# isl-org/adaptive-surface-reconstruction

Hardware: AMD Instinct MI355X
Metric: input points/sec to signed implicit values (higher is better)
Workload: dtype f32 via bf16x3 (24-bit operands, f32 accumulate)

## Files before the change

adaptive-surface-reconstruction_amd/csrc/asr_common.h:

```cpp
#pragma once
#include <hip/hip_runtime.h>

#include <cstdint>
#include <cstdio>
#include <map>
#include <string>
#include <tuple>
#include <vector>

#include "../../include/asr_hip.h"

typedef uint64_t u64;
typedef int64_t i64;
typedef uint32_t u32;

struct Arena {
    struct Slab {
        char* base;
        size_t size, used;
    };
    std::vector<Slab> slabs;
    size_t min_slab = size_t(256) << 20;
    size_t cap = 0;

    void* alloc(size_t bytes) {
        bytes = (bytes + 255) & ~size_t(255);
        if (bytes == 0) bytes = 256;
        for (auto& s : slabs)
            if (s.size - s.used >= bytes) {
                void* p = s.base + s.used;
                s.used += bytes;
                return p;
            }
        size_t sz = bytes > min_slab ? bytes : min_slab;
        if (cap && reserved() + sz > cap) return nullptr;
        void* p = nullptr;
        if (hipMalloc(&p, sz) != hipSuccess) return nullptr;
        slabs.push_back({(char*)p, sz, bytes});
        return p;
    }
    void reset() {
        for (auto& s : slabs) s.used = 0;
    }
    size_t reserved() const {
        size_t t = 0;
        for (auto& s : slabs) t += s.size;
        return t;
    }
    void release() {
        for (auto& s : slabs) (void)hipFree(s.base);
        slabs.clear();
    }
};

struct ArenaMark {
    std::vector<size_t> used;
};
static inline void arena_mark(const Arena& a, ArenaMark& m) {
    m.used.clear();
    for (auto& s : a.slabs) m.used.push_back(s.used);
}
static inline void arena_rewind(Arena& a, const ArenaMark& m) {
    for (size_t i = 0; i < a.slabs.size(); ++i) a.slabs[i].used = i < m.used.size() ? m.used[i] : 0;
}

struct GridDev {
    i64 v = 0, p = 0;
    u64* keys = nullptr;
    float* centers = nullptr;
    float* sizes = nullptr;
    int32_t* nidx = nullptr;
    uint8_t* nkidx = nullptr;
    i64* nrs = nullptr;
    int32_t* up_idx = nullptr;
    uint8_t* up_kidx = nullptr;
    i64* up_rs = nullptr;
    int32_t* down_idx = nullptr;
    uint8_t* down_kidx = nullptr;
    i64* down_rs = nullptr;
    int32_t* perm_nb = nullptr;
    int32_t* perm_up = nullptr;
    int32_t* perm_down = nullptr;
};

struct AsrOptions {
    i64 sconv_min_blocks = 2816;
    i64 sconv16_min_blocks = 1024;
    i64 sconv_wide_min = 2048;
    i64 row_segment = 524288;
    i64 search_hash_level = -1;
    i64 knn_deep = 1;
    i64 knn_cells = 1;
    i64 plan_arena = 0;
    i64 sconv_plan = 1;
    i64 row_ranked = 1;
    i64 row_lpt = 1;
    i64 overlap = 1;
    i64 cconv_valu = 0;
    i64 build_search = 1;
    i64 shard_geometry = -1;
    i64 shard_timing = 0;
    i64 search_priority = 2;
    i64 search_half = 1;
    i64 early_cells = 1;
    i64 early_sort = 1;
    i64 arena_cap_mb = 0;
    i64 inject_failure = 0;
    i64 sconv_split_min_rows = 2048;
    i64 sconv_split_rows = 32768;
};

struct asr_conv_plan_view {
    const uint4* hdr;
    const int32_t* pool;
    i64 groups;
    unsigned pool_bytes;
};
struct asr_conv_plan {
    uint4* hdr = nullptr;
    int32_t* pool = nullptr;
    i64 groups = 0, groups_pad = 0, blocks = 0;
    i64* offs = nullptr;
    const int32_t* nidx = nullptr;
    const uint8_t* kidx = nullptr;
    const i64* rs = nullptr;
    const int32_t* perm = nullptr;
    i64 num_out = 0;
    int K = 0;
    bool usable() const { return hdr && blocks * 64 < (i64(1) << 32) - 65536; }
    asr_conv_plan_view view() const { return {hdr, pool, groups, (unsigned)(blocks * 64)}; }
};

struct AsrPointIndex {
    bool valid = false;
    const float* pts = nullptr;
    const float* radii = nullptr;
    i64 n = 0;
    int lsort = 0;
    float4* sorted = nullptr;
    int32_t* ids = nullptr;
    int32_t* rank = nullptr;
    float* srad = nullptr;
    u64* codes = nullptr;
    u64* tab_keys = nullptr;
    u64 tab_mask = 0;
    int32_t* tab_start = nullptr;
    int32_t* tab_end = nullptr;
    int tab_lmin = 0, tab_lmax = -1, tab_lhash = 0, tab_grow = 0;
};

struct asr_hip_context {
    hipStream_t stream = nullptr;
    std::string err;
    AsrOptions opt;
    std::map<const void*, asr_conv_plan> conv_plans;
    std::map<std::string, i64> sconv_launches;
    ArenaMark build_mark;
    bool build_mark_ok = false;
    Arena persist;
    Arena scratch;
    Arena plan_arena;
    uint64_t plan_arena_epoch = 0;
    u64* nodes = nullptr;
    u64* leaves = nullptr;
    i64 num_nodes = 0, num_leaves = 0;
    asr_octree_frame frame;
    asr_implicit_sizes sizes;
    GridDev grids[ASR_NUM_GRIDS];
    int32_t* agg_idx = nullptr;
    float* agg_dist = nullptr;
    float* agg_compat = nullptr;
    i64* agg_rs = nullptr;
    int32_t* agg_spos = nullptr;
    const float4* agg_sorted = nullptr;
    bool has_search = false;
    bool build_sharded = false;
    const int32_t* agg_rows = nullptr;
    i64 agg_nq = 0;
    const float* agg_qcenters = nullptr;
    const float* agg_qsizes = nullptr;
    AsrPointIndex pindex;
    i64 shard_prefix_hint = 0;
    int search_extras = 0;
    int leaf_lmin = -1, leaf_lmax = -1;
    float* values = nullptr;
    float* feats1 = nullptr;
    int feats1_width = 0;
    float* importance = nullptr;
    float* code = nullptr;
    bool code_ok = false;
    int code_width = 0;
    int code_scale_sdf = 0;
    float stage_ms[6] = {0, 0, 0, 0, 0, 0};
    hipEvent_t ev[8] = {};
    bool ev_ok = false;
    int* d_flags = nullptr;
    int* d_flags_base = nullptr;
    int flags_next = 0;
    float* d_zeros = nullptr;
    float* split_part = nullptr;
    size_t split_part_bytes = 0;
    unsigned* d_status = nullptr;
    unsigned* d_absmax = nullptr;
    void* radius_state = nullptr;
    void* mesh_state = nullptr;
    std::map<std::string, std::pair<const void*, size_t>> named;
    int device = 0;
    asr_hip_context* aux = nullptr;
    bool aux_stream_owned = false;
    hipEvent_t aux_ev = nullptr;
    hipEvent_t aux_t0 = nullptr, aux_t1 = nullptr;
    bool search_overlapped = false;
    typedef std::tuple<const void*, const void*, i64, i64, i64, i64, int> PackedKey;
    std::map<PackedKey, void*> packed_weights;
    Arena shard_mem;
    unsigned* shard_stage_send = nullptr;
    unsigned* shard_stage_recv = nullptr;
    size_t shard_stage_cap = 0;
    struct asr_shard_state* shard = nullptr;
    bool dry_launch = false;
};

#define ASR_FAIL(ctx, code, ...)                         \
    do {                                                 \
        char _b[512];                                    \
        snprintf(_b, sizeof(_b), __VA_ARGS__);           \
        (ctx)->err = _b;                                 \
        return (code);                                   \
    } while (0)

#define ASR_HIP_CHECK(ctx, expr)                                                            \
    do {                                                                                    \
        hipError_t _e = (expr);                                                             \
        if (_e != hipSuccess)                                                               \
            ASR_FAIL(ctx, ASR_HIP_EHIP, "%s failed: %s (%s:%d)", #expr, hipGetErrorString(_e), \
                     __FILE__, __LINE__);                                                   \
    } while (0)

#define ASR_CHECK_LAUNCH(ctx) ASR_HIP_CHECK(ctx, hipGetLastError())

#define ASR_TRY(expr)               \
    do {                            \
        int _r = (expr);            \
        if (_r != ASR_HIP_OK) return _r; \
    } while (0)

static inline int asr_ctx_zeros(asr_hip_context* ctx, const float** out) {
    if (!ctx->d_zeros) {
        ASR_HIP_CHECK(ctx, hipMalloc((void**)&ctx->d_zeros, 4096));
        ASR_HIP_CHECK(ctx, hipMemsetAsync(ctx->d_zeros, 0, 4096, ctx->stream));
    }
    *out = ctx->d_zeros;
    return ASR_HIP_OK;
}

template <class T>
static inline T* arena_alloc(Arena& a, size_t count) {
    return (T*)a.alloc(count * sizeof(T));
}

static inline unsigned grid_for(i64 n, int block) {
    i64 g = (n + block - 1) / block;
    if (g < 1) g = 1;
    return (unsigned)g;
}

__host__ __device__ static inline u64 asr_dilate21(u64 x) {
    x = (x | (x << 32)) & 0x001F00000000FFFFull;
    x = (x | (x << 16)) & 0x00FF0000FF0000FFull;
    x = (x | (x << 8)) & 0xF00F00F00F00F00Full;
    x = (x | (x << 4)) & 0x30C30C30C30C30C3ull;
    x = (x | (x << 2)) & 0x9249249249249249ull;
    return x;
}
__host__ __device__ static inline u64 asr_compact21(u64 x) {
    x &= 0x1249249249249249ull;
    x = ((x >> 2) | x) & 0x30C30C30C30C30C3ull;
    x = ((x >> 4) | x) & 0xF00F00F00F00F00Full;
    x = ((x >> 8) | x) & 0x00FF0000FF0000FFull;
    x = ((x >> 16) | x) & 0x001F00000000FFFFull;
    x = ((x >> 32) | x) & 0x00000000001FFFFFull;
    return x;
}
// ... 190 lines not shown
```

adaptive-surface-reconstruction_amd/csrc/asr_conv16.hip:

```cpp
#include <type_traits>

#include "asr_common.h"

namespace {

typedef float f32x4 __attribute__((ext_vector_type(4)));
typedef unsigned u32x4 __attribute__((ext_vector_type(4)));
typedef _Float16 f16x8 __attribute__((ext_vector_type(8)));
typedef __bf16 bf16x8 __attribute__((ext_vector_type(8)));
typedef float f32x2 __attribute__((ext_vector_type(2)));
typedef __bf16 bf16x2 __attribute__((ext_vector_type(2)));
typedef uint16_t u16;

constexpr int NBR_LD = 57;

constexpr bool is_bf16x3(int mode) { return mode == ASR_CONV16_BF16X3 || mode == ASR_CONV16_BF16X3_2ACC; }

__device__ inline u16 f32_to_bf16_bits(float x) {
    const f32x2 v = {x, 0.f};
    return (u16)(__builtin_bit_cast(unsigned, __builtin_convertvector(v, bf16x2)) & 0xffffu);
}

__device__ inline u16 f32_to_f16_bits(float x) {
    _Float16 h = (_Float16)x;
// ... 422 lines not shown
            if (SV_EXACT || w_lds[s] >= 0) s_B[buf][w_lds[s]] = st[s];
    };
    constexpr int ESZ = MODE == ASR_CONV16_F16 ? 2 : 4;
    const i64 a_span = a.num_inp > 0 ? ((a.num_inp - 1) * a.inp_ld + cin) * ESZ : 0;
    const bool a_big = a_span > (i64)(OOB_OFF - 4096);
    const __amdgpu_buffer_rsrc_t rs_a =
            __builtin_amdgcn_make_buffer_rsrc((void*)a.inp_features, 0, a_big ? 0 : (int)(unsigned)a_span, RSRC_FLAGS);
    const bool cin_tail = cin % KC != 0;
    int cache_k = -2;
    unsigned cache_off = OOB_OFF;
    const char* cache_row = (const char*)zeros;
    bool cache_valid = false;
    auto gather_a = [&](const int qk, const int qp, u32x4 (&aq)[NJ * AW]) __attribute__((always_inline)) {
        if (qk != cache_k) {
            cache_k = qk;
            const int idx = qk < 0 ? -1 : s_nbr[lrow * NBR_LD + qk];
            cache_valid = idx >= 0;
            cache_off = cache_valid ? (unsigned)idx * (unsigned)(a.inp_ld * ESZ) + (unsigned)(8 * g * ESZ) : OOB_OFF;
            if (a_big) cache_row = (const char*)a.inp_features + (i64)(cache_valid ? idx : 0) * a.inp_ld * ESZ;
        }
        if (!a_big && !cin_tail) {
            const int soff = qp * KC * ESZ;
#pragma unroll
            for (int j = 0; j < NJ; ++j)
#pragma unroll
                for (int h = 0; h < AW; ++h)
                    aq[j * AW + h] = __builtin_amdgcn_raw_buffer_load_b128(rs_a, (int)cache_off + (32 * j + 4 * h) * ESZ,
                                                                           soff, 0);
            return;
        }
#pragma unroll
        for (int j = 0; j < NJ; ++j) {
            const int c = qp * KC + 32 * j + 8 * g;
#pragma unroll
            for (int h = 0; h < AW; ++h) {
                const int cc = c + 4 * h;
                if (a_big) {
                    const void* src = (cache_valid && cc < cin) ? (const void*)(cache_row + (i64)cc * ESZ) : (const void*)zeros;
                    aq[j * AW + h] = *reinterpret_cast<const u32x4*>(src);
                } else {
                    const unsigned vo = cc < cin ? cache_off + (unsigned)((32 * j + 4 * h) * ESZ) : OOB_OFF;
                    aq[j * AW + h] = __builtin_amdgcn_raw_buffer_load_b128(rs_a, (int)vo, qp * KC * ESZ, 0);
                }
            }
        }
    };

    unsigned long long todo1 = bmask;
    int k_cur = bmask ? __builtin_ctzll(bmask) : -1, p_cur = 0;
    int k1 = k_cur, p1 = 0;
    ASR_SEQ_ADVANCE(todo1, k1, p1)
    if (k_cur >= 0) {
        load_panel(k_cur, p_cur, stage0);
        gather_a(k_cur, p_cur, a_q0);
        store_panel(0, stage0);
        load_panel(k1, p1, stage1);
        gather_a(k1, p1, a_q1);
    }
    __syncthreads();
    int buf = 0;
    const int ncol = lane & 15;
    auto step = [&](u32x4 (&aq)[NJ * AW], u32x4 (&st_free)[SV], u32x4 (&st_next)[SV]) __attribute__((always_inline)) {
        int k2 = k1, p2 = p1;
        ASR_SEQ_ADVANCE(todo1, k2, p2)
        store_panel(buf ^ 1, st_next);
        load_panel(k2, p2, st_free);
        const bool active = (wmask >> k_cur) & 1;
        float w4[4] = {0.f, 0.f, 0.f, 0.f};
        if (DUAL && has_b && p_cur == npanel - 1 && active) {
#pragma unroll
            for (int i = 0; i < 4; ++i) {
                const int idx = s_nbr[(wave * 16 + 4 * g + i) * NBR_LD + k_cur];
                w4[i] = *(idx >= 0 ? a.inp_importance + idx : zeros);
            }
        }
        u32x4 fa[NJ][PLANES];
        {
#pragma unroll
            for (int j = 0; j < NJ; ++j) {
                if constexpr (MODE == ASR_CONV16_F16) {
                    fa[j][0] = aq[j];
                } else if constexpr (MODE == ASR_CONV16_F16X2) {
                    sconv16_split_f16x2(aq[j * 2], aq[j * 2 + 1], a_scale, fa[j][0], fa[j][PLANES > 1 ? 1 : 0]);
                } else {
                    unsigned p0[4], p1[4], p2[4];
#pragma unroll
                    for (int i = 0; i < 4; ++i) {
                        const f32x2 v = {__uint_as_float(aq[j * 2 + (i >> 1)][2 * (i & 1)]),
                                         __uint_as_float(aq[j * 2 + (i >> 1)][2 * (i & 1) + 1])};
                        p0[i] = __builtin_bit_cast(unsigned, __builtin_convertvector(v, bf16x2));
                        const f32x2 r1 = {v.x - __uint_as_float(p0[i] << 16), v.y - __uint_as_float(p0[i] & 0xffff0000u)};
                        p1[i] = __builtin_bit_cast(unsigned, __builtin_convertvector(r1, bf16x2));
                        const f32x2 r2 = {r1.x - __uint_as_float(p1[i] << 16), r1.y - __uint_as_float(p1[i] & 0xffff0000u)};
                        p2[i] = __builtin_bit_cast(unsigned, __builtin_convertvector(r2, bf16x2));
                    }
                    fa[j][0] = (u32x4){p0[0], p0[1], p0[2], p0[3]};
                    fa[j][PLANES > 1 ? 1 : 0] = (u32x4){p1[0], p1[1], p1[2], p1[3]};
                    fa[j][PLANES > 2 ? 2 : 0] = (u32x4){p2[0], p2[1], p2[2], p2[3]};
                }
            }
        }
        gather_a(k2, p2, aq);
        if (active) {
            const u32x4* sb = s_B[buf];
            __builtin_amdgcn_s_setprio(1);
            sconv16_products<NT, KC, MODE, IMP, DUAL, PLANES, NJ, NL>(fa, sb, acc, tacc, has_b, ncol, g, lo);
            __builtin_amdgcn_s_setprio(0);
            if ((IMP || DUAL) && p_cur == npanel - 1) {
                if (IMP) {
#pragma unroll
                    for (int i = 0; i < 4; ++i) w4[i] = s_w[(wave * 16 + 4 * g + i) * NBR_LD + k_cur];
#pragma unroll
                    for (int nb = 0; nb < NT; ++nb) {
#pragma unroll
                        for (int i = 0; i < 4; ++i) acc[nb][i] += w4[i] * tacc[nb][i];
                        tacc[nb] = {0.f, 0.f, 0.f, 0.f};
                    }
                } else if (has_b) {
#pragma unroll
                    for (int i = 0; i < 4; ++i) acc_b[i] += w4[i] * tacc[0][i];
                    acc[NT - 1] += tacc[0];
                    tacc[0] = {0.f, 0.f, 0.f, 0.f};
                }
            }
        }
        __syncthreads();
        buf ^= 1;
        k_cur = k1;
        p_cur = p1;
        k1 = k2;
        p1 = p2;
    };
    while (k_cur >= 0) {
        step(a_q0, stage0, stage1);
        if (k_cur < 0) break;
        step(a_q1, stage1, stage0);
    }
#undef ASR_SEQ_ADVANCE

    int rows4[4];
    float norms4[4];
#pragma unroll
    for (int i = 0; i < 4; ++i) {
        rows4[i] = s_row[wave * 16 + 4 * g + i];
        norms4[i] = s_norm[wave * 16 + 4 * g + i];
    }
    if constexpr (MODE == ASR_CONV16_BF16X3_2ACC && !IMP) sconv16_fold_lo<NT, DUAL, NL>(acc, lo, tacc[0], has_b);
    sconv16_epilogue<NT, MODE, DUAL>(a, acc, acc_b, rows4, norms4, n0, ncol, ca, cout, has_b, out_f16, zeros, unscale);
    if (a.out_importance && ychunk == 0 && tid < TM && s_row[tid] >= 0)
        a.out_importance[s_row[tid]] = s_norm[tid];
}



constexpr int SPLIT_RANGES = 5;
__host__ __device__ inline unsigned long long split_range_mask(int s) {
    const int lo = s == 0 ? 0 : 7 + 12 * (s - 1), hi = s == 0 ? 7 : 19 + 12 * (s - 1);
    return ((1ull << hi) - 1) ^ ((1ull << lo) - 1);
}
__device__ inline int split_range_of_y(int y) { return y == 0 ? 1 : (y == 1 ? 2 : (y == 2 ? 0 : y)); }
struct asr_split_args {
    float* part;
    i64 stride;
};

#ifndef ASR_PLAN_LINEGATHER
#define ASR_PLAN_LINEGATHER 1
#endif
#ifndef ASR_PLAN_LINEDMA
#define ASR_PLAN_LINEDMA 1
#endif
#ifndef ASR_PLAN_LDMA_DUAL
#define ASR_PLAN_LDMA_DUAL 1
#endif
#ifndef ASR_PLAN_LDMA_F16
#define ASR_PLAN_LDMA_F16 8
#endif
template <int NT, int KC, int WAVES, int MODE, bool IMP, bool DUAL>
constexpr bool plan_ldma() {
    if (MODE == ASR_CONV16_F16)
        return ASR_PLAN_LINEGATHER && ASR_PLAN_LINEDMA && ASR_PLAN_LDMA_F16 && KC == 64 && WAVES == 8 && (IMP || DUAL || NT <= ASR_PLAN_LDMA_F16);
    return ASR_PLAN_LINEGATHER && ASR_PLAN_LINEDMA && KC == 32 && WAVES == 8 &&
           ((!IMP && !DUAL && NT <= 4) || (ASR_PLAN_LDMA_DUAL && (IMP || DUAL)));
}
template <int NT, int KC, int WAVES, int MODE, bool IMP, bool DUAL>
constexpr bool plan_line() {
    return plan_ldma<NT, KC, WAVES, MODE, IMP, DUAL>() ||
           (ASR_PLAN_LINEGATHER && MODE != ASR_CONV16_F16 && KC == 32 && (NT <= 2 || (NT == 4 && WAVES == 8 && (IMP || DUAL))));
}
template <int NT, int KC, int WAVES, int MODE, bool IMP, bool DUAL, bool SPLIT = false>
__global__ __launch_bounds__(WAVES * 64, WAVES == 8 ? (MODE == ASR_CONV16_BF16X3_2ACC ? 4 : (NT >= 8 && (IMP || DUAL) ? 2 : 3)) : 4)
void k_sconv_plan16(
        asr_sparse_conv_args a, asr_conv_plan_view plan, const u16* __restrict__ packed, int cin_pad, int ctot_pad, int out_f16,
        const float* __restrict__ zeros, asr_split_args sp) {
    constexpr int TM = WAVES * 16;
    constexpr int NCOL = NT * 16;
    constexpr int PLANES = is_bf16x3(MODE) ? 3 : (MODE == ASR_CONV16_F16X2 ? 2 : 1);
    constexpr int SLOTS = KC / 8;
    constexpr int NJ = KC / 32;
    constexpr int PV = PLANES * NCOL * SLOTS;
    constexpr int PLANE_PIECES = NCOL * SLOTS;
    constexpr int NCHUNK = PV / 64;
    constexpr int CHUNKS_PER_PLANE = PLANE_PIECES / 64;
    constexpr int SV = (NCHUNK + WAVES - 1) / WAVES;
    constexpr int AW = MODE == ASR_CONV16_F16 ? 1 : 2;
    constexpr int ESZ = MODE == ASR_CONV16_F16 ? 2 : 4;
    constexpr bool ROWW = IMP || DUAL;
    __shared__ __attribute__((aligned(16))) u32x4 s_B0[PV];
    __shared__ __attribute__((aligned(16))) u32x4 s_B1[PV];
    constexpr bool LDMA_ = plan_ldma<NT, KC, WAVES, MODE, IMP, DUAL>();
    __shared__ unsigned long long s_wm_own[LDMA_ ? 1 : WAVES];
    unsigned long long* const s_wm = LDMA_ ? reinterpret_cast<unsigned long long*>(&s_B1[PV - 4]) : s_wm_own;
    __shared__ __attribute__((aligned(16))) u32x4 s_stage[plan_line<NT, KC, WAVES, MODE, IMP, DUAL>() ? WAVES * 128 : 1];

    const int tid = threadIdx.x;
    const int wave = __builtin_amdgcn_readfirstlane(tid >> 6), lane = tid & 63;
    const int nY = ctot_pad / NCOL;
    i64 tile = blockIdx.x;
    int ychunk = 0;
    if (nY > 1) {
        const i64 r8 = blockIdx.x >> 3;
        ychunk = (int)(r8 % nY);
        tile = (r8 / nY) * 8 + (blockIdx.x & 7);
    }
    const i64 row0 = tile * TM;
    if (row0 >= a.num_out) return;
    const int n0 = ychunk * NCOL;
    const int K = a.kernel_size;
    const int cin = a.cin;
    const int ca = a.cout;
    const int cout = a.cout + (DUAL ? a.cout_b : 0);
    const bool has_b = DUAL && ychunk == nY - 1;
    const bool roww = IMP || has_b;
    const int r = lane & 15, g = lane >> 4;
    const int ncol = r;

    const i64 grp = tile * WAVES + wave;
    uint4 h = make_uint4(0, 0, 0, 0);
    if (grp < plan.groups) h = plan.hdr[grp];
    const unsigned long long wmask_all =
            ((unsigned long long)(unsigned)__builtin_amdgcn_readfirstlane((int)h.x) |
             ((unsigned long long)(unsigned)__builtin_amdgcn_readfirstlane((int)h.y) << 32)) & ((1ull << K) - 1);
    const unsigned woff = (unsigned)__builtin_amdgcn_readfirstlane((int)h.z);
    if (lane == 0) s_wm[wave] = wmask_all;
    __syncthreads();
    unsigned long long bmask = 0;
#pragma unroll
    for (int w = 0; w < WAVES; ++w) bmask |= s_wm[w];
    bmask = (unsigned long long)(unsigned)__builtin_amdgcn_readfirstlane((int)(unsigned)bmask) |
            ((unsigned long long)(unsigned)__builtin_amdgcn_readfirstlane((int)(unsigned)(bmask >> 32)) << 32);
    unsigned long long wmask = wmask_all;
    bool partial = false;
    if constexpr (SPLIT) {
        const unsigned long long rm = split_range_mask(split_range_of_y((int)blockIdx.y));
        if ((bmask & rm) == 0) return;
        partial = (bmask & ~rm) != 0;
        wmask &= rm;
        bmask &= rm;
    }

    f32x4 acc[NT];
    constexpr int NL = MODE != ASR_CONV16_BF16X3_2ACC ? NT : (DUAL && NT > 1 ? NT - 1 : NT);
    f32x4 lo[NL];
#pragma unroll
    for (int t = 0; t < NL; ++t) lo[t] = {0.f, 0.f, 0.f, 0.f};
    f32x4 tacc[IMP ? NT : 1];
#pragma unroll
    for (int t = 0; t < NT; ++t) acc[t] = {0.f, 0.f, 0.f, 0.f};
#pragma unroll
    for (int t = 0; t < (IMP ? NT : 1); ++t) tacc[t] = {0.f, 0.f, 0.f, 0.f};
    f32x4 acc_b = {0.f, 0.f, 0.f, 0.f};
    float norm4[4] = {0.f, 0.f, 0.f, 0.f};

    const int npanel = (cin + KC - 1) / KC;
    const i64 plane_stride = (i64)K * ctot_pad * cin_pad;
    float a_scale = 1.f, unscale[2] = {1.f, 1.f};
    if constexpr (MODE == ASR_CONV16_F16X2) {
        const int sa = f16x2_scale_exp(*a.inp_absmax);
        const int un = -(sa + *(const int*)(packed + PLANES * plane_stride));
        a_scale = f16x2_pow2(sa);
        unscale[0] = f16x2_pow2(un / 2);
        unscale[1] = f16x2_pow2(un - un / 2);
    }

    constexpr unsigned OOB_OFF = 0xFFFFE000u;
    const int nslots = __popcll(bmask);
    const int panel_bytes = ctot_pad * KC * 2, slot_bytes = npanel * panel_bytes;
    int v_seq, v_off;
    {
        const bool mine = lane < K && ((bmask >> lane) & 1);
        const int ord = __popcll(bmask & ((1ull << lane) - 1));
        const bool has = (wmask >> lane) & 1;
        const unsigned off = has ? (woff + (unsigned)__popcll(wmask_all & ((1ull << lane) - 1))) * 64u : OOB_OFF;
        const int dst = (mine ? ord : 63) * 4;
        v_seq = __builtin_amdgcn_ds_permute(dst, lane * slot_bytes);
        v_off = __builtin_amdgcn_ds_permute(dst, (int)off);
        if (lane >= nslots) {
            v_seq = 0;
            v_off = (int)OOB_OFF;
        }
    }
#define ASR_SEQ_ADVANCE(i, p)                   \
    {                                           \
        const int nx_ = (p) + 1;                \
        const int wrap_ = nx_ == npanel ? 1 : 0; \
        (p) = wrap_ ? 0 : nx_;                  \
        (i) += wrap_;                           \
    }
    constexpr int RSRC_FLAGS = 0x00020000;
    const __amdgpu_buffer_rsrc_t rs_w =
            __builtin_amdgcn_make_buffer_rsrc((void*)packed, 0, (int)(PLANES * plane_stride * 2), RSRC_FLAGS);
    const __amdgpu_buffer_rsrc_t rs_p =
            __builtin_amdgcn_make_buffer_rsrc((void*)plan.pool, 0, (int)plan.pool_bytes, RSRC_FLAGS);
    const __amdgpu_buffer_rsrc_t rs_i = __builtin_amdgcn_make_buffer_rsrc(
            (void*)(ROWW ? a.inp_importance : zeros), 0, ROWW ? (int)(unsigned)(a.num_inp * 4) : 4, RSRC_FLAGS);
    const int lane16 = lane * 16;
    unsigned w_soff[SV];
#pragma unroll
    for (int s = 0; s < SV; ++s) {
        const int c = s * WAVES + wave;
        const int pl = c / CHUNKS_PER_PLANE, ci = c % CHUNKS_PER_PLANE;
        w_soff[s] = (unsigned)((pl * plane_stride + (i64)n0 * KC) * 2 + ci * 1024);
    }
    auto dma_panel = [&](const int qi, const int qp, auto bufc) __attribute__((always_inline)) {
        const int soff = __builtin_amdgcn_readlane(v_seq, qi & 63) + qp * panel_bytes;
        u32x4* dst = decltype(bufc)::value ? s_B1 : s_B0;
#pragma unroll
        for (int s = 0; s < SV; ++s) {
            const int c = s * WAVES + wave;
            if (NCHUNK % WAVES == 0 || c < NCHUNK)
                __builtin_amdgcn_raw_ptr_buffer_load_lds(rs_w, (__attribute__((address_space(3))) void*)&dst[c * 64], 16,
                                                         lane16, soff + (int)w_soff[s], 0, 0);
        }
    };
    auto lacks = [&](const int i) __attribute__((always_inline)) -> int {
        return (unsigned)__builtin_amdgcn_readlane(v_off, i & 63) == OOB_OFF ? (int)OOB_OFF : 0;
    };
    auto load_idx = [&](const int i) __attribute__((always_inline)) -> int {
        return (int)__builtin_amdgcn_raw_buffer_load_b32(rs_p, r * 4 + lacks(i), __builtin_amdgcn_readlane(v_off, i & 63), 0);
    };
    auto load_idx4 = [&](const int i) __attribute__((always_inline)) -> u32x4 {
        return __builtin_amdgcn_raw_buffer_load_b128(rs_p, g * 16 + lacks(i), __builtin_amdgcn_readlane(v_off, i & 63), 0);
    };
    const __amdgpu_buffer_rsrc_t rs_a = __builtin_amdgcn_make_buffer_rsrc(
            (void*)a.inp_features, 0, (int)(unsigned)(a.num_inp > 0 ? ((a.num_inp - 1) * a.inp_ld + cin) * ESZ : 0),
            RSRC_FLAGS);
    int cache_i = -2;
    unsigned cache_off = OOB_OFF;
    int pref_idx = -1;
    constexpr bool LDMA = plan_ldma<NT, KC, WAVES, MODE, IMP, DUAL>();
    constexpr bool LINE = plan_line<NT, KC, WAVES, MODE, IMP, DUAL>();
    unsigned cache_off1 = OOB_OFF;
    int pref_idx1 = -1;
    const int lrow = lane >> 3, lpiece = lane & 7;
    auto load_idx_row = [&](const int i, const int row) __attribute__((always_inline)) -> int {
        return (int)__builtin_amdgcn_raw_buffer_load_b32(rs_p, row * 4 + lacks(i), __builtin_amdgcn_readlane(v_off, i & 63), 0);
    };
    auto gather_a = [&](const int qi, const int qp, u32x4 (&aq)[NJ * AW], const bool first) __attribute__((always_inline)) {
        const bool sw = qi != cache_i;
        if constexpr (LINE) {
            int idx0 = pref_idx, idx1 = pref_idx1;
            if (first) {
                idx0 = load_idx_row(qi, lrow);
                idx1 = load_idx_row(qi, 8 + lrow);
            }
            if (sw) {
                cache_i = qi;
                const bool has = lacks(qi) == 0;
                const int pc = LDMA ? (lpiece ^ (lrow & 7)) : lpiece;
                cache_off = has && idx0 >= 0 ? (unsigned)idx0 * (unsigned)(a.inp_ld * ESZ) + (unsigned)(pc * 16) : OOB_OFF;
                cache_off1 = has && idx1 >= 0 ? (unsigned)idx1 * (unsigned)(a.inp_ld * ESZ) + (unsigned)(pc * 16) : OOB_OFF;
                pref_idx = load_idx_row(qi + 1, lrow);
                pref_idx1 = load_idx_row(qi + 1, 8 + lrow);
            }
            const int soff = qp * KC * ESZ;
            if constexpr (LDMA) {
                u32x4* st = s_stage + wave * 128;
                __builtin_amdgcn_raw_ptr_buffer_load_lds(rs_a, (__attribute__((address_space(3))) void*)st, 16, (int)cache_off, soff, 0, 0);
                __builtin_amdgcn_raw_ptr_buffer_load_lds(rs_a, (__attribute__((address_space(3))) void*)(st + 64), 16, (int)cache_off1, soff, 0, 0);
            } else {
                aq[0] = __builtin_amdgcn_raw_buffer_load_b128(rs_a, (int)cache_off, soff, 0);
                aq[1] = __builtin_amdgcn_raw_buffer_load_b128(rs_a, (int)cache_off1, soff, 0);
            }
            return;
        }
        int idx = pref_idx;
        if (first) idx = load_idx(qi);
        if (sw) {
            cache_i = qi;
            const bool valid = lacks(qi) == 0 && idx >= 0;
            cache_off = valid ? (unsigned)idx * (unsigned)(a.inp_ld * ESZ) + (unsigned)(8 * g * ESZ) : OOB_OFF;
            pref_idx = load_idx(qi + 1);
        }
        const int soff = qp * KC * ESZ;
#pragma unroll
        for (int j = 0; j < NJ; ++j)
#pragma unroll
            for (int hh = 0; hh < AW; ++hh)
                aq[j * AW + hh] =
                        __builtin_amdgcn_raw_buffer_load_b128(rs_a, (int)cache_off + (32 * j + 4 * hh) * ESZ, soff, 0);
    };

    constexpr int DEPTH = ((WAVES == 8 && !IMP && !DUAL) || LDMA) ? 1 : 2;
    u32x4 a_q0[NJ * AW], a_q1[DEPTH == 2 ? NJ * AW : 1];
    int k_cur = 0, p_cur = 0;
    int k1 = 0, p1 = 0;
    ASR_SEQ_ADVANCE(k1, p1)
    u32x4 idx4_cur = {~0u, ~0u, ~0u, ~0u}, idx4_next = {~0u, ~0u, ~0u, ~0u};
    using B0 = std::integral_constant<int, 0>;
    using B1 = std::integral_constant<int, 1>;
    if (k_cur < nslots) {
        dma_panel(k_cur, p_cur, B0());
        if (ROWW && roww) idx4_next = load_idx4(k_cur);
        gather_a(k_cur, p_cur, a_q0, true);
        if constexpr (DEPTH == 2) gather_a(k1, p1, a_q1, false);
    }
    asm volatile("s_waitcnt vmcnt(0)" ::: "memory");
    __builtin_amdgcn_s_barrier();
    asm volatile("" ::: "memory");
    auto step = [&](u32x4 (&aq)[NJ * AW], auto bufc) __attribute__((always_inline)) {
        constexpr int BUF = decltype(bufc)::value;
        int k2 = k1, p2 = p1;
        ASR_SEQ_ADVANCE(k2, p2)
        if constexpr (LDMA) {
            asm volatile("s_waitcnt vmcnt(0)" ::: "memory");
            const u32x4* st = s_stage + wave * 128;
            aq[0] = st[r * 8 + ((MODE == ASR_CONV16_F16 ? g : 2 * g) ^ (r & 7))];
            aq[1] = st[r * 8 + ((MODE == ASR_CONV16_F16 ? 4 + g : 2 * g + 1) ^ (r & 7))];
            asm volatile("s_waitcnt lgkmcnt(0)" ::: "memory");
        }
        dma_panel(k1, p1, std::integral_constant<int, BUF ^ 1>());
        if constexpr (LDMA && !ROWW) gather_a(k1, p1, aq, false);
        __builtin_amdgcn_sched_barrier(0);
        const bool active = lacks(k_cur) == 0;
        float w4[4] = {0.f, 0.f, 0.f, 0.f};
        const bool slot_end = p_cur == npanel - 1;
        if (ROWW && roww) {
            if (p_cur == 0) idx4_cur = idx4_next;
            if (p1 == 0) idx4_next = load_idx4(k1);
            if (slot_end && active) {
#pragma unroll
                for (int i = 0; i < 4; ++i)
                    w4[i] = __uint_as_float(__builtin_amdgcn_raw_buffer_load_b32(rs_i, (int)(idx4_cur[i] * 4u), 0, 0));
            }
        }
        u32x4 fa[NJ][PLANES];
        if (active) {
            if constexpr (LINE && !LDMA) {
                u32x4* st = s_stage + wave * 128;
                const int wcol = lpiece ^ (lrow & 7);
                st[lrow * 8 + wcol] = aq[0];
                st[(8 + lrow) * 8 + wcol] = aq[1];
                __builtin_amdgcn_wave_barrier();
                aq[0] = st[r * 8 + ((2 * g) ^ (r & 7))];
                aq[1] = st[r * 8 + ((2 * g + 1) ^ (r & 7))];
                __builtin_amdgcn_wave_barrier();
            }
#pragma unroll
            for (int j = 0; j < NJ; ++j) {
                if constexpr (MODE == ASR_CONV16_F16) {
                    fa[j][0] = aq[j];
                } else if constexpr (MODE == ASR_CONV16_F16X2) {
                    sconv16_split_f16x2(aq[j * 2], aq[j * 2 + 1], a_scale, fa[j][0], fa[j][PLANES > 1 ? 1 : 0]);
                } else {
                    unsigned p0[4], p1v[4], p2v[4];
#pragma unroll
                    for (int i = 0; i < 4; ++i) {
                        const f32x2 v = {__uint_as_float(aq[j * 2 + (i >> 1)][2 * (i & 1)]),
                                         __uint_as_float(aq[j * 2 + (i >> 1)][2 * (i & 1) + 1])};
                        p0[i] = __builtin_bit_cast(unsigned, __builtin_convertvector(v, bf16x2));
                        const f32x2 r1 = {v.x - __uint_as_float(p0[i] << 16), v.y - __uint_as_float(p0[i] & 0xffff0000u)};
                        p1v[i] = __builtin_bit_cast(unsigned, __builtin_convertvector(r1, bf16x2));
                        const f32x2 r2 = {r1.x - __uint_as_float(p1v[i] << 16), r1.y - __uint_as_float(p1v[i] & 0xffff0000u)};
                        p2v[i] = __builtin_bit_cast(unsigned, __builtin_convertvector(r2, bf16x2));
                    }
                    fa[j][0] = (u32x4){p0[0], p0[1], p0[2], p0[3]};
                    fa[j][PLANES > 1 ? 1 : 0] = (u32x4){p1v[0], p1v[1], p1v[2], p1v[3]};
                    fa[j][PLANES > 2 ? 2 : 0] = (u32x4){p2v[0], p2v[1], p2v[2], p2v[3]};
                }
            }
        }
        if constexpr (DEPTH == 2)
            gather_a(k2, p2, aq, false);
        else if constexpr (!LDMA || ROWW)
            gather_a(k1, p1, aq, false);
        if (active) {
            const u32x4* sb = BUF ? s_B1 : s_B0;
            __builtin_amdgcn_s_setprio(1);
            sconv16_products<NT, KC, MODE, IMP, DUAL, PLANES, NJ, NL>(fa, sb, acc, tacc, has_b, ncol, g, lo);
            __builtin_amdgcn_s_setprio(0);
            if (ROWW && roww && slot_end) {
#pragma unroll
                for (int i = 0; i < 4; ++i) norm4[i] += w4[i];
                if (IMP) {
#pragma unroll
                    for (int nb = 0; nb < NT; ++nb) {
#pragma unroll
                        for (int i = 0; i < 4; ++i) acc[nb][i] += w4[i] * tacc[nb][i];
                        tacc[nb] = {0.f, 0.f, 0.f, 0.f};
                    }
                } else {
#pragma unroll
                    for (int i = 0; i < 4; ++i) acc_b[i] += w4[i] * tacc[0][i];
                    acc[NT - 1] += tacc[0];
                    tacc[0] = {0.f, 0.f, 0.f, 0.f};
                }
            }
        }
        asm volatile("s_waitcnt vmcnt(%0)" ::"n"(NJ * AW) : "memory");
        __builtin_amdgcn_s_barrier();
        asm volatile("" ::: "memory");
        k_cur = k1;
        p_cur = p1;
        k1 = k2;
        p1 = p2;
    };
    while (k_cur < nslots) {
        step(a_q0, B0());
        if (k_cur >= nslots) break;
        if constexpr (DEPTH == 2)
            step(a_q1, B1());
        else
            step(a_q0, B1());
    }
#undef ASR_SEQ_ADVANCE

    if constexpr (MODE == ASR_CONV16_BF16X3_2ACC && !IMP) sconv16_fold_lo<NT, DUAL, NL>(acc, lo, tacc[0], has_b);
    int q4[4];
#pragma unroll
    for (int i = 0; i < 4; ++i) {
        const i64 lr = row0 + wave * 16 + 4 * g + i;
        q4[i] = lr < a.num_out ? (a.row_perm ? a.row_perm[lr] : (int)lr) : -1;
    }
    if constexpr (SPLIT) {
        if (partial) {
            float* pr = sp.part + (i64)split_range_of_y((int)blockIdx.y) * sp.stride;
#pragma unroll
            for (int i = 0; i < 4; ++i) {
                const i64 lr = row0 + wave * 16 + 4 * g + i;
#pragma unroll
                for (int nb = 0; nb < NT; ++nb)
                    pr[lr * ctot_pad + n0 + nb * 16 + ncol] = acc[nb][i] * unscale[0] * unscale[1];
            }
            return;
        }
    }
    sconv16_epilogue<NT, MODE, DUAL>(a, acc, acc_b, q4, norm4, n0, ncol, ca, cout, has_b, out_f16, zeros, unscale);
    if (ROWW && a.out_importance && ncol == 0 && (DUAL ? has_b : ychunk == 0)) {
#pragma unroll
        for (int i = 0; i < 4; ++i)
            if (q4[i] >= 0) a.out_importance[q4[i]] = norm4[i];
    }
}

template <int WAVES>
__global__ __launch_bounds__(256) void k_sconv_split_reduce(asr_sparse_conv_args a, asr_conv_plan_view plan, asr_split_args sp,
                                                            int ctot_pad, const float* __restrict__ zeros) {
    constexpr int TM = WAVES * 16;
    const i64 tile = blockIdx.x / WAVES;
    const int grp_in_tile = (int)(blockIdx.x % WAVES);
    unsigned long long bmask = 0;
    for (int w = 0; w < WAVES; ++w) {
        const i64 grp = tile * WAVES + w;
        if (grp < plan.groups) {
            const uint4 h = plan.hdr[grp];
            bmask |= (unsigned long long)h.x | ((unsigned long long)h.y << 32);
        }
    }
    bmask &= (1ull << a.kernel_size) - 1;
    int ranges = 0;
#pragma unroll
    for (int s = 0; s < SPLIT_RANGES; ++s) ranges += (bmask & split_range_mask(s)) != 0;
    if (ranges < 2) return;
    const int c4n = ctot_pad / 4;
    unsigned amax = 0;
    const bool res_v4 = a.residual && a.residual_ld % 4 == 0 && ((uintptr_t)a.residual & 15) == 0;
    const bool out_v4 = a.out_ld % 4 == 0 && ((uintptr_t)a.out & 15) == 0;
    for (int e = threadIdx.x; e < 16 * c4n; e += blockDim.x) {
        const int r = e / c4n, c = 4 * (e % c4n);
        const i64 lr = tile * TM + grp_in_tile * 16 + r;
        if (lr >= a.num_out) break;
        const i64 q = a.row_perm ? a.row_perm[lr] : lr;
        float4 pv[SPLIT_RANGES];
#pragma unroll
        for (int s = 0; s < SPLIT_RANGES; ++s)
            if (bmask & split_range_mask(s)) pv[s] = *reinterpret_cast<const float4*>(sp.part + s * sp.stride + lr * ctot_pad + c);
        float4 v = make_float4(0.f, 0.f, 0.f, 0.f);
        bool first = true;
#pragma unroll
        for (int s = 0; s < SPLIT_RANGES; ++s) {
            if (!(bmask & split_range_mask(s))) continue;
            if (first) {
                v = pv[s];
                first = false;
            } else {
                v.x += pv[s].x;
                v.y += pv[s].y;
                v.z += pv[s].z;
                v.w += pv[s].w;
            }
        }
        float o[4] = {v.x, v.y, v.z, v.w};
        float4 res = make_float4(0.f, 0.f, 0.f, 0.f);
        const bool full4 = c + 3 < a.cout;
        if (res_v4 && full4) res = *reinterpret_cast<const float4*>(a.residual + q * a.residual_ld + c);
        const float rr[4] = {res.x, res.y, res.z, res.w};
#pragma unroll
        for (int i = 0; i < 4; ++i) {
            const int col = c + i;
            if (col >= a.cout) continue;
            float x = o[i] + (a.bias ? a.bias[col] : 0.f);
            if (a.relu) x = fmaxf(x, 0.f);
            if (a.residual) x += (res_v4 && full4) ? rr[i] : a.residual[q * a.residual_ld + col];
            o[i] = x;
            amax = max(amax, __float_as_uint(x) & 0x7fffffffu);
        }
        if (full4 && out_v4) {
            *reinterpret_cast<float4*>(a.out + q * a.out_ld + c) = make_float4(o[0], o[1], o[2], o[3]);
        } else {
#pragma unroll
            for (int i = 0; i < 4; ++i)
                if (c + i < a.cout) a.out[q * a.out_ld + c + i] = o[i];
        }
    }
    if (a.out_absmax) {
#pragma unroll
        for (int o = 32; o > 0; o >>= 1) amax = max(amax, (unsigned)__shfl_xor((int)amax, o, 64));
        if ((threadIdx.x & 63) == 0 && amax > __hip_atomic_load(a.out_absmax, __ATOMIC_RELAXED, __HIP_MEMORY_SCOPE_AGENT))
            atomicMax(a.out_absmax, amax);
    }
}


}

static inline int round_up(int x, int m) { return (x + m - 1) / m * m; }

static inline int panel_depth(int mode, int cin) { return mode == ASR_CONV16_F16 && round_up(cin, 32) % 64 == 0 ? 64 : 32; }

static inline bool mode_ok(int mode) { return mode == ASR_CONV16_F16 || is_bf16x3(mode) || mode == ASR_CONV16_F16X2; }

size_t asr_conv16_packed_bytes(int mode, int K, int cin, int cout, int cout_b) {
    const size_t planes = is_bf16x3(mode) ? 3 : (mode == ASR_CONV16_F16X2 ? 2 : 1);
    return planes * (size_t)K * round_up(cout + cout_b, 16) * round_up(cin, 32) * sizeof(u16) +
           (mode == ASR_CONV16_F16X2 ? 16 : 0);
}

int asr_conv16_absmax(asr_hip_context* ctx, const float* x, i64 rows, int c, i64 ld, unsigned* out) {
    ASR_HIP_CHECK(ctx, hipMemsetAsync(out, 0, sizeof(unsigned), ctx->stream));
    const i64 total = rows * c;
    if (total <= 0) return ASR_HIP_OK;
    k_absmax<<<(unsigned)std::min<i64>((total + 255) / 256, 8192), 256, 0, ctx->stream>>>(x, rows, c, ld, out);
    ASR_CHECK_LAUNCH(ctx);
    return ASR_HIP_OK;
}

int asr_conv16_pack(asr_hip_context* ctx, int mode, const float* wa, const float* wb, int K, int cin, int ca, int cb,
                    void* out) {
    if (!mode_ok(mode))
        ASR_FAIL(ctx, ASR_HIP_EINVAL,
                 "sparse_conv_pack: mode must be ASR_CONV16_F16, ASR_CONV16_BF16X3, ASR_CONV16_F16X2 or ASR_CONV16_BF16X3_2ACC");
    if (!wa || !out || K < 1 || K > 56 || cin < 1 || ca < 1 || cb < 0 || (cb > 0 && !wb))
        ASR_FAIL(ctx, ASR_HIP_EINVAL, "sparse_conv_pack: bad argument");
    const int cin_pad = round_up(cin, 32), ctot_pad = round_up(ca + cb, 16);
    const i64 total = (i64)K * ctot_pad * cin_pad;
    unsigned* w_absmax = nullptr;
    if (mode == ASR_CONV16_F16X2) {
        w_absmax = (unsigned*)((u16*)out + 2 * total) + 1;
        ASR_TRY(asr_conv16_absmax(ctx, wa, (i64)K * cin, ca, ca, w_absmax));
        if (cb > 0) {
            k_absmax<<<(unsigned)std::min<i64>(((i64)K * cin * cb + 255) / 256, 8192), 256, 0, ctx->stream>>>(
                    wb, (i64)K * cin, cb, cb, w_absmax);
            ASR_CHECK_LAUNCH(ctx);
        }
    }
    k_pack_filters<<<(unsigned)std::min<i64>((total + 255) / 256, 65535), 256, 0, ctx->stream>>>(
            wa, wb, K, cin, ca, cb, cin_pad, ctot_pad, mode, panel_depth(mode, cin), (u16*)out, w_absmax);
    ASR_CHECK_LAUNCH(ctx);
    return ASR_HIP_OK;
}

int asr_conv16_convert(asr_hip_context* ctx, const void* in, i64 n, void* out, int to_f16) {
    if (n <= 0) return ASR_HIP_OK;
    if (to_f16)
        k_f32_to_f16<<<grid_for(n, 256), 256, 0, ctx->stream>>>((const float*)in, n, (u16*)out);
    else
        k_f16_to_f32<<<grid_for(n, 256), 256, 0, ctx->stream>>>((const u16*)in, n, (float*)out);
    ASR_CHECK_LAUNCH(ctx);
    return ASR_HIP_OK;
}

int asr_conv_sparse16(asr_hip_context* ctx, const asr_sparse_conv_args* pa, const void* packed, int mode,
                      int out_f16, const asr_conv_plan* plan) {
    asr_sparse_conv_args a = *pa;
    if (a.num_out <= 0) return ASR_HIP_OK;
    if (!mode_ok(mode)) ASR_FAIL(ctx, ASR_HIP_EINVAL, "sparse_conv16: unknown mode");
    if (mode != ASR_CONV16_F16 && out_f16) ASR_FAIL(ctx, ASR_HIP_EINVAL, "sparse_conv16: bf16x3, bf16x3_2acc and f16x2 write f32");
    if (a.kernel_size < 1 || a.kernel_size > 56) ASR_FAIL(ctx, ASR_HIP_EINVAL, "sparse_conv16: kernel_size must be 1..56");
    const bool dual = a.cout_b > 0;
    const bool imp = a.inp_importance || a.neighbors_importance;
    const int esz = mode == ASR_CONV16_F16 ? 2 : 4;
    const int gran = 16 / esz;
    if (a.cin % gran != 0 || a.inp_ld % gran != 0 || (uintptr_t)a.inp_features % 16 != 0 || (uintptr_t)packed % 16 != 0)
        ASR_FAIL(ctx, ASR_HIP_EINVAL, "sparse_conv16: cin and the row stride must be multiples of %d, 16-byte rows", gran);
    if (dual && (!a.inp_importance || a.neighbors_importance || a.cout % 16 != 8 || a.cout_b != 8 || a.residual))
        ASR_FAIL(ctx, ASR_HIP_EINVAL,
                 "sparse_conv16: second filter bank needs inp_importance (per input row), cout %% 16 == 8, cout_b == 8");
    if (a.inp_ld < a.cin || a.out_ld < a.cout + a.cout_b)
        ASR_FAIL(ctx, ASR_HIP_EINVAL, "sparse_conv16: row stride smaller than channel count");
    const float* zeros = nullptr;
    ASR_TRY(asr_ctx_zeros(ctx, &zeros));
    if (mode == ASR_CONV16_F16X2 && !a.inp_absmax) {
        if (!ctx->d_absmax) ASR_HIP_CHECK(ctx, hipMalloc((void**)&ctx->d_absmax, 256 * sizeof(unsigned)));
        unsigned* m = ctx->d_absmax + 255;
        ASR_TRY(asr_conv16_absmax(ctx, a.inp_features, a.num_inp, a.cin, a.inp_ld, m));
        a.inp_absmax = m;
    }
    const int cin_pad = round_up(a.cin, 32), ctot_pad = round_up(a.cout + a.cout_b, 16);
    int nt = 8;
    while (nt > 1 && ctot_pad % (nt * 16) != 0) nt >>= 1;
    const i64 tiles64 = (a.num_out + 63) / 64;
    if (a.force_nt) {
        if ((a.force_nt != 1 && a.force_nt != 2 && a.force_nt != 4 && a.force_nt != 8) || ctot_pad % (a.force_nt * 16) != 0)
            ASR_FAIL(ctx, ASR_HIP_EINVAL, "sparse_conv16: force_nt must be 1, 2, 4 or 8 and divide the padded width");
        nt = a.force_nt;
    } else {
        while (nt > 2 && tiles64 * (ctot_pad / (nt * 16)) < ctx->opt.sconv16_min_blocks) nt >>= 1;
    }
    const i64 tiles128 = (a.num_out + 127) / 128;
    bool wide = tiles128 * (ctot_pad / (nt * 16)) >= ctx->opt.sconv_wide_min;
    if (a.force_waves) {
        if (a.force_waves != 4 && a.force_waves != 8) ASR_FAIL(ctx, ASR_HIP_EINVAL, "sparse_conv16: force_waves must be 4 or 8");
        wide = a.force_waves == 8;
    }
    const bool kc64 = panel_depth(mode, a.cin) == 64;
    const bool use_plan = plan && plan->usable() && ctx->opt.sconv_plan && !a.neighbors_importance &&
                          !(a.normalize && !imp) && !(a.out_importance && !imp) &&
                          a.num_inp * a.inp_ld * esz < (i64(1) << 32) - 65536 && a.cin % (kc64 ? 64 : 32) == 0;
    asr_conv_plan_view pv = {nullptr, nullptr, 0, 0};
    if (use_plan) {
        if (plan->num_out != a.num_out || plan->K < a.kernel_size || plan->perm != a.row_perm)
            ASR_FAIL(ctx, ASR_HIP_EINVAL, "sparse_conv16: the plan was built for another list");
        pv = plan->view();
    }
    const bool split = use_plan && !dual && !imp && mode != ASR_CONV16_F16 && a.kernel_size == 55 && !a.force_nt &&
                       !a.force_waves && ctot_pad % 64 == 0 && ctx->opt.sconv_split_rows > 0 &&
                       a.num_inp <= ctx->opt.sconv_split_rows && a.num_inp >= ctx->opt.sconv_split_min_rows;
    asr_split_args spa = {nullptr, 0};
    if (split) {
        nt = ctot_pad % 128 == 0 ? 8 : 4;
        wide = true;
        const i64 tiles = (a.num_out + 127) / 128;
        spa.stride = tiles * 128 * ctot_pad;
        const size_t need = (size_t)SPLIT_RANGES * spa.stride * sizeof(float);
        if (need > ctx->split_part_bytes) {
            if (ctx->split_part) {
                ASR_HIP_CHECK(ctx, hipStreamSynchronize(ctx->stream));
                (void)hipFree(ctx->split_part);
                ctx->split_part = nullptr;
                ctx->split_part_bytes = 0;
            }
            ASR_HIP_CHECK(ctx, hipMalloc((void**)&ctx->split_part, need + need / 4));
            ctx->split_part_bytes = need + need / 4;
        }
        spa.part = ctx->split_part;
    }
    if (ctx->dry_launch) return ASR_HIP_OK;
#define ASR_L16(NT_, KC_, W_, M_, I_, D_)                                                                        \
    {                                                                                                            \
        const i64 tiles_ = (a.num_out + W_ * 16 - 1) / (W_ * 16);                                                \
        const i64 ny_ = ctot_pad / (NT_ * 16);                                                                   \
        dim3 grid((unsigned)(ny_ > 1 ? ((tiles_ + 7) / 8) * 8 * ny_ : tiles_));                                  \
        if (use_plan)                                                                                            \
            k_sconv_plan16<NT_, KC_, W_, M_, I_, D_><<<grid, dim3(W_ * 64), 0, ctx->stream>>>(                   \
                    a, pv, (const u16*)packed, cin_pad, ctot_pad, out_f16, zeros, spa);                          \
        else                                                                                                     \
            k_sconv_mfma16<NT_, KC_, W_, M_, I_, D_><<<grid, dim3(W_ * 64), 0, ctx->stream>>>(                   \
                    a, (const u16*)packed, cin_pad, ctot_pad, out_f16, zeros);                                   \
    }
#define ASR_L16_ID(NT_, KC_, W_, M_) \
    if (dual)                        \
        ASR_L16(NT_, KC_, W_, M_, false, true) \
    else if (imp)                    \
        ASR_L16(NT_, KC_, W_, M_, true, false) \
    else                             \
        ASR_L16(NT_, KC_, W_, M_, false, false)
#define ASR_L16_W(NT_, KC_, M_) \
    if (wide)                   \
        ASR_L16_ID(NT_, KC_, 8, M_) \
    else                        \
        ASR_L16_ID(NT_, KC_, 4, M_)
#define ASR_L16_NT(KC_, M_)                 \
    switch (nt) {                           \
        case 8: ASR_L16_W(8, KC_, M_) break; \
        case 4: ASR_L16_W(4, KC_, M_) break; \
        case 2: ASR_L16_W(2, KC_, M_) break; \
        default: ASR_L16_W(1, KC_, M_) break; \
    }
#define ASR_L16_SPLIT(NT_, M_)                                                                                   \
    {                                                                                                            \
        const i64 tiles_ = (a.num_out + 127) / 128;                                                              \
        const i64 ny_ = ctot_pad / (NT_ * 16);                                                                   \
        dim3 grid((unsigned)(ny_ > 1 ? ((tiles_ + 7) / 8) * 8 * ny_ : tiles_), SPLIT_RANGES);                    \
        k_sconv_plan16<NT_, 32, 8, M_, false, false, true><<<grid, dim3(512), 0, ctx->stream>>>(                 \
                a, pv, (const u16*)packed, cin_pad, ctot_pad, out_f16, zeros, spa);                              \
        ASR_CHECK_LAUNCH(ctx);                                                                                   \
        k_sconv_split_reduce<8><<<dim3((unsigned)(tiles_ * 8)), dim3(256), 0, ctx->stream>>>(a, pv, spa, ctot_pad, zeros); \
    }
    if (split) {
        if (mode == ASR_CONV16_F16X2) {
            if (nt == 8)
                ASR_L16_SPLIT(8, ASR_CONV16_F16X2)
            else
                ASR_L16_SPLIT(4, ASR_CONV16_F16X2)
        } else if (mode == ASR_CONV16_BF16X3_2ACC) {
            if (nt == 8)
                ASR_L16_SPLIT(8, ASR_CONV16_BF16X3_2ACC)
            else
                ASR_L16_SPLIT(4, ASR_CONV16_BF16X3_2ACC)
        } else {
            if (nt == 8)
                ASR_L16_SPLIT(8, ASR_CONV16_BF16X3)
            else
                ASR_L16_SPLIT(4, ASR_CONV16_BF16X3)
        }
    } else if (mode == ASR_CONV16_F16) {
        if (kc64)
            ASR_L16_NT(64, ASR_CONV16_F16)
        else
            ASR_L16_NT(32, ASR_CONV16_F16)
    } else if (mode == ASR_CONV16_F16X2) {
        ASR_L16_NT(32, ASR_CONV16_F16X2)
    } else if (mode == ASR_CONV16_BF16X3_2ACC) {
        ASR_L16_NT(32, ASR_CONV16_BF16X3_2ACC)
    } else {
        ASR_L16_NT(32, ASR_CONV16_BF16X3)
    }
#undef ASR_L16_SPLIT
#undef ASR_L16_NT
#undef ASR_L16_W
#undef ASR_L16_ID
#undef ASR_L16
    ASR_CHECK_LAUNCH(ctx);
    {
        char key[64];
        snprintf(key, sizeof(key), "%d,%d,%d,%d,%d,%d,%d%s", nt, kc64 ? 64 : 32, imp && !dual ? 1 : 0, wide ? 8 : 4,
                 dual ? 1 : 0, mode, use_plan ? 1 : 0, split ? ",1" : "");
        ++ctx->sconv_launches[key];
    }
    return ASR_HIP_OK;
}
```

Measured before the change: 274.2 million.

## Precompute per-neighbor importance weights into a plan-aligned pool before conv

Adds a pre-pass kernel that gathers input importance values into a float pool laid out like the plan's neighbor-index pool. The conv kernel then loads one weight per lane from that pool and spreads it across lanes with ds_bpermute, replacing the old scheme of loading index quads and issuing dependent gathers at slot end. This removes a serial index-then-importance load chain from the inner loop, at the cost of an extra launch and scratch memory sized to the pool. The arena is rewound right after allocation, so the buffer may be reused by later allocations while still in use.

```diff
diff --git a/adaptive-surface-reconstruction_amd/csrc/asr_common.h b/adaptive-surface-reconstruction_amd/csrc/asr_common.h
--- a/adaptive-surface-reconstruction_amd/csrc/asr_common.h
+++ b/adaptive-surface-reconstruction_amd/csrc/asr_common.h
@@ -115,6 +115,7 @@
     const int32_t* pool;
     i64 groups;
     unsigned pool_bytes;
+    const float* wpool;
 };
 struct asr_conv_plan {
     uint4* hdr = nullptr;
@@ -128,7 +129,7 @@
     i64 num_out = 0;
     int K = 0;
     bool usable() const { return hdr && blocks * 64 < (i64(1) << 32) - 65536; }
-    asr_conv_plan_view view() const { return {hdr, pool, groups, (unsigned)(blocks * 64)}; }
+    asr_conv_plan_view view() const { return {hdr, pool, groups, (unsigned)(blocks * 64), nullptr}; }
 };
 
 struct AsrPointIndex {
diff --git a/adaptive-surface-reconstruction_amd/csrc/asr_conv16.hip b/adaptive-surface-reconstruction_amd/csrc/asr_conv16.hip
--- a/adaptive-surface-reconstruction_amd/csrc/asr_conv16.hip
+++ b/adaptive-surface-reconstruction_amd/csrc/asr_conv16.hip
@@ -598,6 +598,21 @@
 }
 
 
+
+__global__ __launch_bounds__(256) void k_sconv_wpool(const int4* __restrict__ pool, const i64* __restrict__ offs, i64 groups_pad,
+                                                    i64 blocks, const float* __restrict__ imp, unsigned num_inp,
+                                                    float4* __restrict__ wpool) {
+    const i64 lo = max(offs[0], (i64)0) * 4, hi = min(offs[groups_pad], blocks) * 4;
+    for (i64 t = lo + (i64)blockIdx.x * blockDim.x + threadIdx.x; t < hi; t += (i64)gridDim.x * blockDim.x) {
+        const int4 i = pool[t];
+        float4 w;
+        w.x = (unsigned)i.x < num_inp ? imp[i.x] : 0.f;
+        w.y = (unsigned)i.y < num_inp ? imp[i.y] : 0.f;
+        w.z = (unsigned)i.z < num_inp ? imp[i.z] : 0.f;
+        w.w = (unsigned)i.w < num_inp ? imp[i.w] : 0.f;
+        wpool[t] = w;
+    }
+}
 
 constexpr int SPLIT_RANGES = 5;
 __host__ __device__ inline unsigned long long split_range_mask(int s) {
@@ -759,7 +774,7 @@
     const __amdgpu_buffer_rsrc_t rs_p =
             __builtin_amdgcn_make_buffer_rsrc((void*)plan.pool, 0, (int)plan.pool_bytes, RSRC_FLAGS);
     const __amdgpu_buffer_rsrc_t rs_i = __builtin_amdgcn_make_buffer_rsrc(
-            (void*)(ROWW ? a.inp_importance : zeros), 0, ROWW ? (int)(unsigned)(a.num_inp * 4) : 4, RSRC_FLAGS);
+            (void*)(ROWW ? plan.wpool : zeros), 0, ROWW ? (int)plan.pool_bytes : 4, RSRC_FLAGS);
     const int lane16 = lane * 16;
     unsigned w_soff[SV];
 #pragma unroll
@@ -785,8 +800,8 @@
     auto load_idx = [&](const int i) __attribute__((always_inline)) -> int {
         return (int)__builtin_amdgcn_raw_buffer_load_b32(rs_p, r * 4 + lacks(i), __builtin_amdgcn_readlane(v_off, i & 63), 0);
     };
-    auto load_idx4 = [&](const int i) __attribute__((always_inline)) -> u32x4 {
-        return __builtin_amdgcn_raw_buffer_load_b128(rs_p, g * 16 + lacks(i), __builtin_amdgcn_readlane(v_off, i & 63), 0);
+    auto load_w = [&](const int i) __attribute__((always_inline)) -> unsigned {
+        return __builtin_amdgcn_raw_buffer_load_b32(rs_i, r * 4 + lacks(i), __builtin_amdgcn_readlane(v_off, i & 63), 0);
     };
     const __amdgpu_buffer_rsrc_t rs_a = __builtin_amdgcn_make_buffer_rsrc(
             (void*)a.inp_features, 0, (int)(unsigned)(a.num_inp > 0 ? ((a.num_inp - 1) * a.inp_ld + cin) * ESZ : 0),
@@ -852,12 +867,12 @@
     int k_cur = 0, p_cur = 0;
     int k1 = 0, p1 = 0;
     ASR_SEQ_ADVANCE(k1, p1)
-    u32x4 idx4_cur = {~0u, ~0u, ~0u, ~0u}, idx4_next = {~0u, ~0u, ~0u, ~0u};
+    unsigned w_cur = 0u, w_next = 0u;
     using B0 = std::integral_constant<int, 0>;
     using B1 = std::integral_constant<int, 1>;
     if (k_cur < nslots) {
         dma_panel(k_cur, p_cur, B0());
-        if (ROWW && roww) idx4_next = load_idx4(k_cur);
+        if (ROWW && roww) w_next = load_w(k_cur);
         gather_a(k_cur, p_cur, a_q0, true);
         if constexpr (DEPTH == 2) gather_a(k1, p1, a_q1, false);
     }
@@ -881,14 +896,9 @@
         const bool active = lacks(k_cur) == 0;
         float w4[4] = {0.f, 0.f, 0.f, 0.f};
         const bool slot_end = p_cur == npanel - 1;
-        if (ROWW && roww) {
-            if (p_cur == 0) idx4_cur = idx4_next;
-            if (p1 == 0) idx4_next = load_idx4(k1);
-            if (slot_end && active) {
-#pragma unroll
-                for (int i = 0; i < 4; ++i)
-                    w4[i] = __uint_as_float(__builtin_amdgcn_raw_buffer_load_b32(rs_i, (int)(idx4_cur[i] * 4u), 0, 0));
-            }
+        if (ROWW && roww && slot_end) {
+            w_cur = w_next;
+            w_next = load_w(k1);
         }
         u32x4 fa[NJ][PLANES];
         if (active) {
@@ -936,6 +946,9 @@
             sconv16_products<NT, KC, MODE, IMP, DUAL, PLANES, NJ, NL>(fa, sb, acc, tacc, has_b, ncol, g, lo);
             __builtin_amdgcn_s_setprio(0);
             if (ROWW && roww && slot_end) {
+#pragma unroll
+                for (int i = 0; i < 4; ++i)
+                    w4[i] = __uint_as_float((unsigned)__builtin_amdgcn_ds_bpermute((20 * g + i) * 4, (int)w_cur));
 #pragma unroll
                 for (int i = 0; i < 4; ++i) norm4[i] += w4[i];
                 if (IMP) {
@@ -1183,7 +1196,7 @@
     const bool use_plan = plan && plan->usable() && ctx->opt.sconv_plan && !a.neighbors_importance &&
                           !(a.normalize && !imp) && !(a.out_importance && !imp) &&
                           a.num_inp * a.inp_ld * esz < (i64(1) << 32) - 65536 && a.cin % (kc64 ? 64 : 32) == 0;
-    asr_conv_plan_view pv = {nullptr, nullptr, 0, 0};
+    asr_conv_plan_view pv = {nullptr, nullptr, 0, 0, nullptr};
     if (use_plan) {
         if (plan->num_out != a.num_out || plan->K < a.kernel_size || plan->perm != a.row_perm)
             ASR_FAIL(ctx, ASR_HIP_EINVAL, "sparse_conv16: the plan was built for another list");
@@ -1211,7 +1224,23 @@
         }
         spa.part = ctx->split_part;
     }
+    float4* wpool = nullptr;
+    if (use_plan && (dual || imp)) {
+        ArenaMark before;
+        arena_mark(ctx->scratch, before);
+        wpool = arena_alloc<float4>(ctx->scratch, (size_t)plan->blocks * 4);
+        if (!wpool) ASR_FAIL(ctx, ASR_HIP_EHIP, "arena allocation failed");
+        arena_rewind(ctx->scratch, before);
+        pv.wpool = (const float*)wpool;
+    }
     if (ctx->dry_launch) return ASR_HIP_OK;
+    if (wpool && plan->blocks > 0) {
+        const i64 n4 = std::min<i64>(plan->blocks, plan->groups_pad * (i64)plan->K) * 4;
+        k_sconv_wpool<<<(unsigned)std::min<i64>(grid_for(n4, 256), 2048), 256, 0, ctx->stream>>>(
+                (const int4*)plan->pool, plan->offs, plan->groups_pad, plan->blocks, a.inp_importance,
+                (unsigned)std::min<i64>(a.num_inp, 0x7fffffff), wpool);
+        ASR_CHECK_LAUNCH(ctx);
+    }
 #define ASR_L16(NT_, KC_, W_, M_, I_, D_)                                                                        \
     {                                                                                                            \
         const i64 tiles_ = (a.num_out + W_ * 16 - 1) / (W_ * 16);                                                \
```

Result: no change. 273.3 million (-0.3%).
